# microsoft/CoCosNet

Measured on AMD Instinct MI355X. Metric: images/sec fwd+bwd ADE20k 256x256 batch-8/GPU (correspondence hot path), higher is better.
Workload: dtype f32 (K2 products as 3-term f16 hi/lo split on the f16 MFMA, fp32 accumulate); 1 GPU; ADE20k 256x256 batch 8/GPU, 64x64 grid (HW=4096), K=256, Cv=154 (rgb+151 labels), match_kernel 1, PONO_C, T=0.01; precision=f16x3; scope=hotpath: theta/phi 1x1 conv + centre/L2norm + fused corr-softmax-warp fwd+bwd; global_batch=8, parallelism=dp1, grad_payload=path, grad_allreduce_bytes=0

## Files before the change

### cocosnet_amd/csrc/split_f16.hip

```cpp
#include "common.h"

namespace cocos {

typedef _Float16 f16x4 __attribute__((ext_vector_type(4)));
typedef _Float16 f16x8 __attribute__((ext_vector_type(8)));

__device__ __forceinline__ void split1(float x, _Float16& hi, _Float16& lo) {
    hi = (_Float16)x;
    lo = (_Float16)(x - (float)hi);
}

__device__ __forceinline__ float scale_from_amax(float amax);

__global__ __launch_bounds__(256) void split_f16_flat_kernel(const float* __restrict__ x,
                                                             _Float16* __restrict__ hi,
                                                             _Float16* __restrict__ lo, size_t n4, size_t n,
                                                             float scale, const float* __restrict__ amax_dev,
                                                             float* __restrict__ scale_out) {
    const size_t i = (size_t)blockIdx.x * 256 + threadIdx.x;
    if (amax_dev) {
        scale = scale_from_amax(*amax_dev);
        if (scale_out && i == 0) *scale_out = scale;
    }
    if (i < n4) {
// ... 66 lines not shown
                if (c0 + cbase + e < Cpad) { hrow[c0 + cbase + e] = h[e]; lrow[c0 + cbase + e] = l[e]; }
        }
    }
}

__global__ __launch_bounds__(256) void split_f16_transpose_kernel(const float* __restrict__ x, _Float16* __restrict__ hi,
                                                                  _Float16* __restrict__ lo, int C, int N, int Cpad, float scale,
                                                                  const float* __restrict__ amax_dev,
                                                                  float* __restrict__ scale_out) {
    split_f16_transpose_tile(x, hi, lo, C, N, Cpad, scale, amax_dev, scale_out, blockIdx.z);
}

struct SplitPair {
    const float* x[2];
    _Float16 *hi[2], *lo[2];
    const float* amax[2];
    float* scale_out[2];
};
__global__ __launch_bounds__(256) void split_f16_transpose_pair_kernel(const SplitPair sp, int B, int C, int N, int Cpad) {
    const bool second = (int)blockIdx.z >= B;
    split_f16_transpose_tile(second ? sp.x[1] : sp.x[0], second ? sp.hi[1] : sp.hi[0], second ? sp.lo[1] : sp.lo[0], C, N, Cpad, 1.0f,
                             second ? sp.amax[1] : sp.amax[0], second ? sp.scale_out[1] : sp.scale_out[0],
                             (int)blockIdx.z - (second ? B : 0));
}

}

namespace cocos {

__global__ __launch_bounds__(256) void split_f16_rows_kernel(const float* __restrict__ x, _Float16* __restrict__ hi,
                                                             _Float16* __restrict__ lo, int rows, int cols,
                                                             int cols_pad, float scale,
                                                             const float* __restrict__ amax_dev,
                                                             float* __restrict__ scale_out) {
    const size_t i = (size_t)blockIdx.x * 256 + threadIdx.x;
    if (amax_dev) {
        scale = scale_from_amax(*amax_dev);
        if (scale_out && i == 0) *scale_out = scale;
    }
    if (i >= (size_t)rows * cols_pad) return;
    const int r = (int)(i / cols_pad), c = (int)(i - (size_t)r * cols_pad);
    _Float16 a = (_Float16)0.f, b = (_Float16)0.f;
    if (c < cols) split1(x[(size_t)r * cols + c] * scale, a, b);
    hi[i] = a;
    lo[i] = b;
}
// ... 63 lines not shown

extern "C" int cocos_split_f16_transpose_pair(const float* x0, void* hi0, void* lo0, const float* amax0_dev, float* scale0_out_dev,
                                              const float* x1, void* hi1, void* lo1, const float* amax1_dev, float* scale1_out_dev,
                                              int B, int C, int N, int Cpad, cocos_stream_t stream) {
    using namespace cocos;
    COCOS_REQUIRE(x0 && hi0 && lo0 && amax0_dev && scale0_out_dev && x1 && hi1 && lo1 && amax1_dev && scale1_out_dev, COCOS_ERR_INVALID,
                  "split_f16_transpose_pair: null pointer");
    COCOS_REQUIRE(B >= 1 && C >= 1 && N >= 1 && 2 * B <= 65535 && Cpad >= C && (Cpad + 63) / 64 <= 65535, COCOS_ERR_INVALID,
                  "split_f16_transpose_pair: bad dims B=%d C=%d N=%d Cpad=%d", B, C, N, Cpad);
    for (const void* p : {(const void*)hi0, (const void*)lo0, (const void*)hi1, (const void*)lo1})
        COCOS_REQUIRE(aligned16(p), COCOS_ERR_INVALID, "split_f16_transpose_pair: planes must be 16-byte aligned");
    SplitPair sp;
    sp.x[0] = x0; sp.x[1] = x1;
    sp.hi[0] = static_cast<_Float16*>(hi0); sp.hi[1] = static_cast<_Float16*>(hi1);
    sp.lo[0] = static_cast<_Float16*>(lo0); sp.lo[1] = static_cast<_Float16*>(lo1);
    sp.amax[0] = amax0_dev; sp.amax[1] = amax1_dev;
    sp.scale_out[0] = scale0_out_dev; sp.scale_out[1] = scale1_out_dev;
    hipLaunchKernelGGL(split_f16_transpose_pair_kernel, dim3((N + 63) / 64, (Cpad + 63) / 64, 2 * B), dim3(256), 0, as_stream(stream), sp,
                       B, C, N, Cpad);
    COCOS_HIP_CHECK(hipGetLastError());
    return COCOS_OK;
}

extern "C" int cocos_split_f16_rows(const float* x, void* hi, void* lo, int rows, int cols, int cols_pad, float scale,
                                    const float* amax_dev, float* scale_out_dev, cocos_stream_t stream) {
    using namespace cocos;
    COCOS_REQUIRE(x && hi && lo, COCOS_ERR_INVALID, "split_f16_rows: null pointer");
    COCOS_REQUIRE(rows >= 1 && cols >= 1 && cols_pad >= cols, COCOS_ERR_INVALID,
                  "split_f16_rows: bad dims rows=%d cols=%d cols_pad=%d", rows, cols, cols_pad);
    const size_t n = (size_t)rows * cols_pad;
    COCOS_REQUIRE((n + 255) / 256 <= 0x7fffffffull, COCOS_ERR_UNSUPPORTED, "split_f16_rows: tensor too large");
    hipLaunchKernelGGL(split_f16_rows_kernel, dim3((unsigned)((n + 255) / 256)), dim3(256), 0, as_stream(stream), x,
                       static_cast<_Float16*>(hi), static_cast<_Float16*>(lo), rows, cols, cols_pad, scale, amax_dev,
                       scale_out_dev);
    COCOS_HIP_CHECK(hipGetLastError());
    return COCOS_OK;
}

extern "C" int cocos_f16_plane_block_mask(const void* plane, int B, int C, int N, unsigned* mask_inout_dev,
                                          cocos_stream_t stream) {
    using namespace cocos;
    COCOS_REQUIRE(plane && mask_inout_dev, COCOS_ERR_INVALID, "f16_plane_block_mask: null pointer");
    COCOS_REQUIRE(B >= 1 && C >= 1 && C <= 1024 && N >= 1 && (long long)B * C <= 0x7fffffffll, COCOS_ERR_INVALID,
                  "f16_plane_block_mask: bad dims B=%d C=%d N=%d (C <= 1024)", B, C, N);
    hipLaunchKernelGGL(f16_plane_block_mask_kernel, dim3((unsigned)(B * C)), dim3(256), 0, as_stream(stream),
                       static_cast<const _Float16*>(plane), C, N, mask_inout_dev);
// ... 4 lines not shown
```

### cocosnet_amd/csrc/warp_values.hip

```cpp
#include <algorithm>

#include "common.h"

namespace cocos {

__global__ __launch_bounds__(256) void warp_values_kernel(const float* __restrict__ img, const float* __restrict__ seg,
                                                          float* __restrict__ out, int Ci, int Cs, int h, int w, int d,
                                                          size_t n, bool vec4, unsigned* __restrict__ amax) {
  float vmax = 0.f;
  const size_t stride = (size_t)gridDim.x * 256;
  const int W = w * d, H = h * d;
  constexpr int U = 4;
  for (size_t i0 = (size_t)blockIdx.x * 256 + threadIdx.x; i0 < n; i0 += stride * U) {
    float v[U];
    const float* pimg[U];
    bool is_img[U], live[U];
#pragma unroll
    for (int u = 0; u < U; ++u) {
      const size_t i = i0 + (size_t)u * stride;
      live[u] = i < n;
      const size_t ii = live[u] ? i : 0;
      const int x = (int)(ii % w);
      size_t r = ii / w;
      const int y = (int)(r % h);
      r /= h;
      const int c = (int)(r % (Ci + Cs));
      const size_t b = r / (Ci + Cs);
      is_img[u] = c < Ci;
      pimg[u] = nullptr;
      v[u] = 0.f;
      if (!is_img[u]) {
        v[u] = seg[((b * Cs + (c - Ci)) * H + (size_t)y * d) * W + (size_t)x * d];
      } else {
        pimg[u] = img + ((b * Ci + c) * H + (size_t)y * d) * W + (size_t)x * d;
      }
    }
#pragma unroll
    for (int u = 0; u < U; ++u) {
      if (is_img[u]) {
        const float* p = pimg[u];
        float acc = 0.f;
        if (vec4) {
#pragma unroll
          for (int a = 0; a < 4; ++a) {
            const f32x4 q = *reinterpret_cast<const f32x4*>(p + (size_t)a * W);
            acc += (q[0] + q[1]) + (q[2] + q[3]);
          }
        } else {
          for (int a = 0; a < d; ++a)
            for (int e = 0; e < d; ++e) acc += p[(size_t)a * W + e];
        }
        v[u] = acc / (float)(d * d);
      }
      if (live[u]) {
        out[i0 + (size_t)u * stride] = v[u];
        vmax = fmaxf(vmax, fabsf(v[u]));
      }
    }
  }
  if (amax) {
      __shared__ float red[4];
      vmax = wave_max_dpp(vmax);
      if ((threadIdx.x & 63) == 0) red[threadIdx.x >> 6] = vmax;
      __syncthreads();
      if (threadIdx.x == 0) atomicMax(amax, __float_as_uint(fmaxf(fmaxf(red[0], red[1]), fmaxf(red[2], red[3]))));
  }
}

__global__ __launch_bounds__(256) void warp_values_patch_kernel(const float* __restrict__ img, const float* __restrict__ seg,
                                                                float* __restrict__ out, int Ci, int Cs, int h, int w, int d,
                                                                size_t n, unsigned* __restrict__ amax) {
  float vmax = 0.f;
  const size_t stride = (size_t)gridDim.x * 256;
  const int W = w * d, H = h * d, Cp = Ci * d * d;
  for (size_t i = (size_t)blockIdx.x * 256 + threadIdx.x; i < n; i += stride) {
    const int x = (int)(i % w);
    size_t r = i / w;
    const int y = (int)(r % h);
    r /= h;
    const int c = (int)(r % (Cp + Cs));
    const size_t b = r / (Cp + Cs);
    float v;
    if (c < Cp) {
      const int cc = c / (d * d), ij = c - cc * d * d, a = ij / d, e = ij - a * d;
      v = img[((b * Ci + cc) * H + (size_t)y * d + a) * W + (size_t)x * d + e];
    } else {
      v = seg[((b * Cs + (c - Cp)) * H + (size_t)y * d) * W + (size_t)x * d];
    }
    out[i] = v;
    vmax = fmaxf(vmax, fabsf(v));
  }
  if (amax) {
      __shared__ float red[4];
      vmax = wave_max_dpp(vmax);
      if ((threadIdx.x & 63) == 0) red[threadIdx.x >> 6] = vmax;
      __syncthreads();
      if (threadIdx.x == 0) atomicMax(amax, __float_as_uint(fmaxf(fmaxf(red[0], red[1]), fmaxf(red[2], red[3]))));
  }
}

}

static int warp_values_impl(const float* img, const float* seg, float* out, int B, int Ci, int Cs, int H, int W, int down,
                            float* amax_inout_dev, cocos_stream_t stream) {
    using namespace cocos;
    COCOS_REQUIRE(out && (img || Ci == 0) && (seg || Cs == 0), COCOS_ERR_INVALID, "warp_values: null pointer");
    COCOS_REQUIRE(B >= 1 && Ci >= 0 && Cs >= 0 && Ci + Cs >= 1 && H >= 1 && W >= 1 && down >= 1, COCOS_ERR_INVALID,
                  "warp_values: bad dims B=%d Ci=%d Cs=%d H=%d W=%d down=%d", B, Ci, Cs, H, W, down);
    COCOS_REQUIRE(H % down == 0 && W % down == 0, COCOS_ERR_UNSUPPORTED,
                  "warp_values: %dx%d is not a multiple of down=%d", H, W, down);
    const size_t n = (size_t)B * (Ci + Cs) * (H / down) * (W / down);
    COCOS_REQUIRE((n + 255) / 256 <= 0x7fffffffull, COCOS_ERR_UNSUPPORTED, "warp_values: tensor too large");
    const bool vec4 = down == 4 && W % 4 == 0 && img && aligned16(img);
    const size_t blocks = std::min<size_t>(1024, (n + 1023) / 1024);
    hipLaunchKernelGGL(warp_values_kernel, dim3((unsigned)blocks), dim3(256), 0, as_stream(stream), img, seg,
                       out, Ci, Cs, H / down, W / down, down, n, vec4, reinterpret_cast<unsigned*>(amax_inout_dev));
    COCOS_HIP_CHECK(hipGetLastError());
    return COCOS_OK;
}

extern "C" int cocos_warp_values(const float* img, const float* seg, float* out, int B, int Ci, int Cs, int H, int W,
                                 int down, cocos_stream_t stream) {
    return warp_values_impl(img, seg, out, B, Ci, Cs, H, W, down, nullptr, stream);
}

extern "C" int cocos_warp_values_amax(const float* img, const float* seg, float* out, int B, int Ci, int Cs, int H, int W,
                                      int down, float* amax_inout_dev, cocos_stream_t stream) {
    COCOS_REQUIRE(amax_inout_dev, COCOS_ERR_INVALID, "warp_values_amax: null amax cell");
    return warp_values_impl(img, seg, out, B, Ci, Cs, H, W, down, amax_inout_dev, stream);
}

extern "C" int cocos_warp_values_patch_amax(const float* img, const float* seg, float* out, int B, int Ci, int Cs, int H, int W,
                                            int down, float* amax_inout_dev, cocos_stream_t stream) {
    using namespace cocos;
    COCOS_REQUIRE(out && (img || Ci == 0) && (seg || Cs == 0), COCOS_ERR_INVALID, "warp_values_patch: null pointer");
    COCOS_REQUIRE(B >= 1 && Ci >= 0 && Cs >= 0 && Ci + Cs >= 1 && H >= 1 && W >= 1 && down >= 1 && down <= 64, COCOS_ERR_INVALID,
                  "warp_values_patch: bad dims B=%d Ci=%d Cs=%d H=%d W=%d down=%d", B, Ci, Cs, H, W, down);
    COCOS_REQUIRE(H % down == 0 && W % down == 0, COCOS_ERR_UNSUPPORTED,
                  "warp_values_patch: %dx%d is not a multiple of down=%d", H, W, down);
    const size_t n = (size_t)B * ((size_t)Ci * down * down + Cs) * (H / down) * (W / down);
    COCOS_REQUIRE((size_t)Ci * down * down + Cs <= 0x7fffffffull && (n + 255) / 256 <= 0x7fffffffull, COCOS_ERR_UNSUPPORTED,
                  "warp_values_patch: tensor too large");
    const size_t blocks = std::min<size_t>(2048, (n + 255) / 256);
    hipLaunchKernelGGL(warp_values_patch_kernel, dim3((unsigned)blocks), dim3(256), 0, as_stream(stream), img, seg, out, Ci, Cs,
                       H / down, W / down, down, n, reinterpret_cast<unsigned*>(amax_inout_dev));
    COCOS_HIP_CHECK(hipGetLastError());
    return COCOS_OK;
}
```

### cocosnet_amd/ops.py

```python
from __future__ import annotations

import ctypes
import os
import sys
import threading
import weakref

import torch

from . import _lib

_C = _lib.CONSTANTS
CENTER_POSITIONS, CENTER_CHANNELS, CENTER_NONE = _C["COCOS_CENTER_POSITIONS"], _C["COCOS_CENTER_CHANNELS"], _C["COCOS_CENTER_NONE"]
NORM_EPS = sys.float_info.epsilon
MAX_FUSED_CV = 160
MAX_FUSED_SPLIT_CV = 159
MAX_DS_WORKSPACE_BYTES = 16 << 30
MAX_SAVED_LOGITS_BYTES = int(os.environ.get("COCOS_MAX_SAVED_LOGITS_BYTES", 16 << 30))
RECOMPUTE_CHUNK_BYTES = int(os.environ.get("COCOS_RECOMPUTE_CHUNK_BYTES", 1 << 30))
BWD_D_PRECOMPUTED = True
FUSED_K = 256
PRECISION = os.environ.get("COCOS_PRECISION", "f16x3")
PROJ_PRECISION = os.environ.get("COCOS_PROJ_PRECISION", "f16x3")
VALUE_LO_SKIP = True
FWD_QK_AHEAD = bool(_lib.CONSTANTS["COCOS_FWD_QK_AHEAD_DEFAULT"])
PROJ_STREAM = True
SPLIT_OPERAND_SCALE = 16.0
MATCH_FUSED = True


def _stream():
    return torch.cuda.current_stream().cuda_stream


def _select_fwd_schedule():
    _lib.load().cocos_corr_fwd_f16x3_qk_ahead(1 if FWD_QK_AHEAD else 0)


class KernelTimer:

    active = None

    def __init__(self, tags=None):
        self.events = {}
        self.tags = None if tags is None else frozenset(tags)

    def __enter__(self):
        KernelTimer.active = self
# ... 207 lines not shown
    shape = (B, N, C) if transpose else (B, C, N)
    hi = torch.empty(shape, device=x.device, dtype=torch.float16)
    lo = torch.empty(shape, device=x.device, dtype=torch.float16)
    _call("split_f16", "cocos_split_f16", x.data_ptr(), hi.data_ptr(), lo.data_ptr(), B, C, N, int(bool(transpose)),
          float(scale), _stream())
    return hi, lo


def split_f16_chan_mask(x: torch.Tensor, amax: torch.Tensor, want_mask: bool):
    x = _chk(x, "split_f16_chan_mask: x")
    B, C, N = x.shape
    if N % 4 != 0 or C > 1024 or x.data_ptr() % 16 != 0:
        hi, lo, sc = split_f16(x, False, amax=amax)
        return hi, lo, sc, (f16_plane_block_mask(lo) if want_mask else None)
    hi = torch.empty((B, C, N), device=x.device, dtype=torch.float16)
    lo = torch.empty((B, C, N), device=x.device, dtype=torch.float16)
    sc = torch.empty(1, device=x.device, dtype=torch.float32)
    mask = _zero_cell(x.device) if want_mask else None
    _call("split_f16", "cocos_split_f16_chan_mask", x.data_ptr(), hi.data_ptr(), lo.data_ptr(), B, C, N, amax.data_ptr(),
          sc.data_ptr(), _ptr(mask), _stream())
    return hi, lo, sc, mask


def f16_plane_block_mask(plane: torch.Tensor) -> torch.Tensor:
    B, C, N = plane.shape
    cell = _zero_cell(plane.device)
    _call("f16_plane_block_mask", "cocos_f16_plane_block_mask", plane.data_ptr(), B, C, N, cell.data_ptr(), _stream())
    return cell


def _recompute_chunk(B, Nq, Nk):
    per_key = max(B * Nq * 4, 1)
    nchunks = max(1, -(-(per_key * Nk) // max(RECOMPUTE_CHUNK_BYTES, 1)))
    kc = max(128, -(-Nk // nchunks) // 128 * 128 + (128 if (-(-Nk // nchunks)) % 128 else 0))
    return min(kc, (Nk + 127) // 128 * 128)


def _saves_logits(B, Nq, Nk) -> bool:
    return (B * Nq * Nk * 4 <= MAX_SAVED_LOGITS_BYTES
            and _lib.load().cocos_corr_softmax_warp_saved_logits_bytes(1, Nq, Nk) < 2 ** 31 - 1)


def _split_bwd_ok(B, Nq, Nk, Cv):
    if not (Nk % 8 == 0 and Nq % 8 == 0 and Cv <= MAX_FUSED_CV):
        return False
    if _saves_logits(B, Nq, Nk):
# ... 11 lines not shown
    while bmode == 2 and tiles * S < GEMM_SPLIT_K_BELOW and S < 8 and Kred % (64 * S) == 0:
        S *= 2
    if S == 1:
        _call(timer, "cocos_hgemm_f16x3", ah.data_ptr(), al.data_ptr(), bh.data_ptr(), bl.data_ptr(), out.data_ptr(), B, M, n, Kred,
              host, _ptr(dev1), _ptr(dev2), bmode, st)
        return
    a2h = ah.view(B, M, S, Kred // S).transpose(1, 2).contiguous()
    a2l = al.view(B, M, S, Kred // S).transpose(1, 2).contiguous()
    part = torch.empty((B, S, M, n), device=out.device, dtype=torch.float32)
    _call(timer, "cocos_hgemm_f16x3", a2h.data_ptr(), a2l.data_ptr(), bh.data_ptr(), bl.data_ptr(), part.data_ptr(), B * S, M, n,
          Kred // S, host, _ptr(dev1), _ptr(dev2), bmode, st)
    torch.sum(part, dim=1, out=out)


def _key_gemm(qch, qcl, dsh, dsl, dk, n, Nq, k_active, qks, ds_scale, gemm_b, st):
    K = dk.shape[1]
    assert qch.shape[1] == K and (not k_active or k_active == K)
    _hgemm_planes("corr_softmax_warp_bwd_key_from_ds", qch, qcl, dsh, dsl, dk, K, n, Nq, 1.0 if qks else 1.0 / SPLIT_OPERAND_SCALE,
                  ds_scale, qks[0] if qks else None, gemm_b, st)


class _CorrSoftmaxWarp(torch.autograd.Function):
    @staticmethod
    def forward(ctx, qn, kn, v, inv_temperature: float, keep_logits: bool, planes=None):
        qn, kn, v = _chk(qn, "qn"), _chk(kn, "kn"), _chk(v, "v")
        B, K, Nq = qn.shape
        Bk, Kk, Nk = kn.shape
        Bv, Cv, Nv = v.shape
        if (Bk, Kk) != (B, K) or (Bv, Nv) != (B, Nk):
            raise ValueError(f"corr_softmax_warp: shape mismatch qn{tuple(qn.shape)} "
                             f"kn{tuple(kn.shape)} v{tuple(v.shape)}")
        out = torch.empty((B, Cv, Nq), device=qn.device, dtype=torch.float32)
        lse = torch.empty((B, Nq), device=qn.device, dtype=torch.float32)
        logits_t = None
        ctx.split = planes is not None
        ctx.v_amax = None
        ctx.v_lomask = None
        if planes is not None:
            qh, ql, kh, kl, vh, vl, v_scale, v_amax, v_lomask = planes[:9]
            qk_scales = planes[13] if len(planes) > 13 else None
            ctx.k_active = planes[14] if len(planes) > 14 else 0
            Kp = FUSED_K if ctx.k_active else K
            ctx.recompute = bool(keep_logits) and not _saves_logits(B, Nq, Nk)
            if keep_logits and not ctx.recompute:
                nbytes = _lib.load().cocos_corr_softmax_warp_saved_logits_bytes(B, Nq, Nk)
                logits_t = torch.empty(nbytes // 4, device=qn.device, dtype=torch.float32)
            ctx.rowstat = torch.empty((B, 3, Nq), device=qn.device, dtype=torch.float32) if (qk_scales and keep_logits) else None
            ctx.mtile = (torch.empty((B, (Nk + 31) // 32, 2, Nq), device=qn.device, dtype=torch.float32)
                         if (qk_scales and logits_t is not None) else None)
            _select_fwd_schedule()
            _call("corr_softmax_warp_fwd", "cocos_corr_softmax_warp_fwd_f16x3_ex", qh.data_ptr(), ql.data_ptr(),
                  kh.data_ptr(), kl.data_ptr(), vh.data_ptr(), vl.data_ptr(), out.data_ptr(), lse.data_ptr(),
                  _ptr(logits_t), v_scale.data_ptr(), _ptr(v_lomask), B, Kp, Nq, Nk, Cv, float(inv_temperature),
                  SPLIT_OPERAND_SCALE, _ptr(qk_scales[0] if qk_scales else None), _ptr(qk_scales[1] if qk_scales else None),
                  _ptr(ctx.rowstat), _ptr(ctx.mtile), ctx.k_active, _stream())
            ctx.v_amax = v_amax
            ctx.v_lomask = v_lomask
            ctx.qk_scales = qk_scales
        else:
            keep = (keep_logits and B * Nq * Nk * 4 <= MAX_DS_WORKSPACE_BYTES and Nq * Nk * 4 < 2 ** 31 - 1)
            logits_t = torch.empty((B, Nk, Nq), device=qn.device, dtype=torch.float32) if keep else None
            _call("corr_softmax_warp_fwd", "cocos_corr_softmax_warp_fwd", qn.data_ptr(), kn.data_ptr(),
                  v.data_ptr(), out.data_ptr(), lse.data_ptr(), _ptr(logits_t), B, K, Nq, Nk, Cv,
                  float(inv_temperature), _stream())
        ctx.save_for_backward(qn, kn, v, out, lse)
        ctx.logits_t = logits_t
        ctx.inv_t = float(inv_temperature)
        recompute = planes is not None and getattr(ctx, "recompute", False)
        ctx.cplanes = planes[9:13] if (planes is not None and len(planes) > 9 and (logits_t is not None or recompute)) else None
        ctx.pplanes = planes[0:4] if recompute else None
        return out

    @staticmethod
    def backward(ctx, dout):
        qn, kn, v, out, lse = ctx.saved_tensors
        dout = _chk(dout, "dout")
        B, K, Nq = qn.shape
        Nk, Cv = kn.shape[2], v.shape[1]
        need_q, need_k, need_v = ctx.needs_input_grad[:3]
        dqn = torch.empty_like(qn) if need_q else None
        dkn = torch.empty_like(kn) if (need_k or need_v) else None
        dv = torch.empty_like(v) if need_v else None
        st = _stream()
        logits_t = ctx.logits_t
        if ctx.split and getattr(ctx, "recompute", False):
            return _CorrSoftmaxWarp._backward_recompute(ctx, qn, kn, v, out, lse, dout, dqn, dkn, dv, need_k)
        if ctx.split and logits_t is not None:
            qch, qcl, kch, kcl = ctx.cplanes
            qks = ctx.qk_scales
            cvp = (Cv + 31) // 32 * 32
            g_amax, v_amax = _recall_amax(dout), ctx.v_amax
            if g_amax is None:
                g_amax = absmax(dout)
            (gph, gpl, g_scale), (vph, vpl, v_scale) = _split_pair_transposed(dout, g_amax, v, v_amax, cvp)
            half = dict(device=qn.device, dtype=torch.float16)
            want_k = dkn is not None
            dsh = dsl = psh = psl = None
            if want_k:
                dsh, dsl = torch.empty((B, Nk, Nq), **half), torch.empty((B, Nk, Nq), **half)
            if dv is not None:
                psh, psl = torch.empty((B, Nk, Nq), **half), torch.empty((B, Nk, Nq), **half)
            ds_scale = torch.empty(1, device=qn.device, dtype=torch.float32)
            blocked = int(Nk % 128 == 0 and Nq % 32 == 0)
            gemm_b = 2 * blocked
            ka = getattr(ctx, "k_active", 0)
            Kp = FUSED_K if ka else K
            if ka:
                dqn_buf = torch.empty((B, Kp, Nq), device=qn.device, dtype=torch.float32)
                dqn = dqn_buf[:, :K] if dqn is not None else None
            elif dqn is None:
                dqn_buf = torch.empty_like(qn)
            else:
                dqn_buf = dqn
            d_pre = _rowdot_cached(dout, out) if BWD_D_PRECOMPUTED else None
            _call("corr_softmax_warp_bwd_query", "cocos_corr_softmax_warp_bwd_query_f16x3_ex", kch.data_ptr(),
                  kcl.data_ptr(), vph.data_ptr(), vpl.data_ptr(), gph.data_ptr(), gpl.data_ptr(),
                  g_scale.data_ptr(), out.data_ptr(), dout.data_ptr(), lse.data_ptr(), logits_t.data_ptr(),
                  dqn_buf.data_ptr(), _ptr(dsh), _ptr(dsl), _ptr(psh), _ptr(psl), v_amax.data_ptr(),
                  v_scale.data_ptr(), ds_scale.data_ptr(), _ptr(ctx.v_lomask), B, Kp, Nq, Nk, Cv, cvp, ctx.inv_t,
                  SPLIT_OPERAND_SCALE, _ptr(qks[0] if qks else None), _ptr(qks[1] if qks else None), blocked,
                  _ptr(getattr(ctx, "rowstat", None)), _ptr(getattr(ctx, "mtile", None)), _ptr(d_pre), ka, st)
            if want_k:
                _key_gemm(qch, qcl, dsh, dsl, dkn, Nk, Nq, ka, qks, ds_scale, gemm_b, st)
            if dv is not None:
                gch, gcl, _ = split_f16(dout, False, amax=g_amax)
                _hgemm_planes("corr_softmax_warp_bwd_dv", gch, gcl, psh, psl, dv, Cv, Nk, Nq, 1.0 / 16384.0, g_scale, None, gemm_b, st)
            return dqn, (dkn if need_k else None), dv, None, None, None
        ds_bytes = B * Nq * Nk * 4
        via_gemm = (dqn is not None and dkn is not None and dv is None
                    and ds_bytes <= MAX_DS_WORKSPACE_BYTES and Nq * Nk * 4 < 2 ** 31 - 1)
        key_recompute = dkn is not None and not via_gemm
        dvec = None
        if key_recompute or (dqn is not None and logits_t is None):
            dvec = torch.empty((B, Nq), device=qn.device, dtype=torch.float32)
            _call("corr_softmax_warp_bwd_prepare", "cocos_corr_softmax_warp_bwd_prepare",
                  out.data_ptr(), dout.data_ptr(), dvec.data_ptr(), B, Nq, Cv, st)
        dims = (B, K, Nq, Nk, Cv, ctx.inv_t, st)
        ds_t = torch.empty((B, Nk, Nq), device=qn.device, dtype=torch.float32) if via_gemm else None
        if dqn is not None:
            _call("corr_softmax_warp_bwd_query", "cocos_corr_softmax_warp_bwd_query", qn.data_ptr(),
                  kn.data_ptr(), v.data_ptr(), out.data_ptr(), lse.data_ptr(), dout.data_ptr(),
                  _ptr(dvec), _ptr(logits_t), _ptr(dqn), _ptr(ds_t), *dims)
        if via_gemm:
            _call("corr_softmax_warp_bwd_key_from_ds", "cocos_corr_softmax_warp_bwd_key_from_ds",
                  qn.data_ptr(), ds_t.data_ptr(), dkn.data_ptr(), B, K, Nq, Nk, st)
        elif dkn is not None:
            _call("corr_softmax_warp_bwd_key", "cocos_corr_softmax_warp_bwd_key", qn.data_ptr(),
                  kn.data_ptr(), v.data_ptr(), lse.data_ptr(), dout.data_ptr(), dvec.data_ptr(),
                  _ptr(dkn), _ptr(dv), *dims)
        return dqn, (dkn if need_k else None), dv, None, None, None


def _corr_bwd_recompute(ctx, qn, kn, v, out, lse, dout, dqn, dkn, dv, need_k):
    qh, ql, kh, kl = ctx.pplanes
    qch, qcl, kch, kcl = ctx.cplanes
    qks = ctx.qk_scales
    B, K, Nq = qn.shape
    Nk, Cv = kn.shape[2], v.shape[1]
    st = _stream()
    lib = _lib.load()
    cvp = (Cv + 31) // 32 * 32
    g_amax, v_amax = _recall_amax(dout), ctx.v_amax
    if g_amax is None:
        g_amax = absmax(dout)
    gph, gpl, g_scale = split_f16(dout, True, cpad=cvp, amax=g_amax)
    vph, vpl, v_scale = split_f16(v, True, cpad=cvp, amax=v_amax)
    gch = gcl = None
    if dv is not None:
        gch, gcl, _ = split_f16(dout, False, amax=g_amax)
    dev, half = qn.device, dict(device=qn.device, dtype=torch.float16)
    want_k = dkn is not None
    kc = _recompute_chunk(B, Nq, Nk)
    ds_scale = torch.empty(1, device=dev, dtype=torch.float32)
# ... 24 lines not shown
        blocked = int(n % 128 == 0 and Nq % 32 == 0)
        dq_c = torch.empty((B, Kp, Nq), device=dev, dtype=torch.float32)
        _call("corr_softmax_warp_bwd_query", "cocos_corr_softmax_warp_bwd_query_f16x3_ex", kchc.data_ptr(), kclc.data_ptr(),
              vphc.data_ptr(), vplc.data_ptr(), gph.data_ptr(), gpl.data_ptr(), g_scale.data_ptr(), out.data_ptr(), dout.data_ptr(),
              lse.data_ptr(), lg.data_ptr(), dq_c.data_ptr(), _ptr(dsh), _ptr(dsl), _ptr(psh), _ptr(psl), v_amax.data_ptr(),
              v_scale.data_ptr(), ds_scale.data_ptr(), _ptr(ctx.v_lomask), B, Kp, Nq, n, Cv, cvp, ctx.inv_t, SPLIT_OPERAND_SCALE,
              _ptr(qks[0] if qks else None), _ptr(qks[1] if qks else None), blocked, _ptr(rowstat), _ptr(mt), _ptr(d_pre), ka, st)
        del lg
        if ka:
            dq_c = dq_c[:, :K]
        dq_acc = dq_c if dq_acc is None else dq_acc.add_(dq_c)
        if want_k:
            dk_c = dkn if n == Nk else torch.empty((B, K, n), device=dev, dtype=torch.float32)
            _key_gemm(qch, qcl, dsh, dsl, dk_c, n, Nq, ka, qks, ds_scale, 2 * blocked, st)
            if dk_c is not dkn:
                dkn[:, :, k0:k0 + n] = dk_c
        if dv is not None:
            dv_c = dv if n == Nk else torch.empty((B, Cv, n), device=dev, dtype=torch.float32)
            _hgemm_planes("corr_softmax_warp_bwd_dv", gch, gcl, psh, psl, dv_c, Cv, n, Nq, 1.0 / 16384.0, g_scale, None, 2 * blocked, st)
            if dv_c is not dv:
                dv[:, :, k0:k0 + n] = dv_c
    if dqn is not None:
        dqn = dq_acc
    return dqn, (dkn if need_k else None), dv, None, None, None


_CorrSoftmaxWarp._backward_recompute = staticmethod(_corr_bwd_recompute)


def _rowdot(a: torch.Tensor, b: torch.Tensor) -> torch.Tensor:
    B, C, N = a.shape
    d = torch.empty((B, N), device=a.device, dtype=torch.float32)
    _call("rowdot", "cocos_rowdot_f64", a.data_ptr(), b.data_ptr(), d.data_ptr(), B, C, N, _stream())
    return d


def _rowdot_cached(dout: torch.Tensor, out: torch.Tensor):
    ent, _tls.known_rowdot = _tls.known_rowdot, None
    if ent is not None:
        ref, version, out_ptr, d = ent
        src = ref()
        if (src is not None and src.data_ptr() == dout.data_ptr() and src.shape == dout.shape and dout._version == version
                and out.data_ptr() == out_ptr and dout.is_contiguous()):
            return d
    return _rowdot(dout, out)


# ... 37 lines not shown
    if not split and (planes.has(qn) or planes.has(kn)):
        raise _lib.CocosHipError("corr_softmax_warp: qn / kn exist as operand planes only (center_l2norm_planes) but this "
                                 "shape does not take the split-precision kernels")

    qk_made = []

    def qk_planes():
        if not qk_made:
            qa, ka_ = absmax(qn), absmax(kn)
            qh, ql, qs = split_f16(qn, True, cpad=FUSED_K, amax=qa)
            kh, kl, ks = split_f16(kn, True, cpad=FUSED_K, amax=ka_)
            cpl = (None,) * 4
            if keep:
                qch, qcl, _ = split_f16(qn, False, amax=qa)
                kch, kcl, _ = split_f16(kn, False, amax=ka_)
                if K < FUSED_K:
                    pad = lambda t: torch.cat([t, t.new_zeros((B, FUSED_K - K, Nk))], dim=1)
                    kch, kcl = pad(kch), pad(kcl)
                cpl = (qch, qcl, kch, kcl)
            qk_made.append((qh, ql, kh, kl, *cpl, (qs, ks), K if K < FUSED_K else 0))
        return qk_made[0]

    def run(vv):
        pl = None
        if split:
            with torch.no_grad():
                v_amax = _recall_amax(vv)
                if v_amax is None:
                    v_amax = absmax(vv)
                vh, vl, v_scale, v_lomask = split_f16_chan_mask(vv, v_amax, VALUE_LO_SKIP and vv.shape[1] > 32 and not operand_amax)
                if operand_amax:
                    pl = (*qk_planes()[:4], vh, vl, v_scale, v_amax, v_lomask, *qk_planes()[4:])
                else:
                    pl = (*planes.get(qn, True, SPLIT_OPERAND_SCALE), *planes.get(kn, True, SPLIT_OPERAND_SCALE),
                          vh, vl, v_scale, v_amax, v_lomask)
                    if keep:
                        pl += (*planes.get(qn, False, SPLIT_OPERAND_SCALE), *planes.get(kn, False, SPLIT_OPERAND_SCALE))
        return _CorrSoftmaxWarp.apply(qn, kn, vv, inv_temperature, keep, pl)

    limit = MAX_FUSED_SPLIT_CV if split else MAX_FUSED_CV
    if Cv <= limit:
        return run(v)
    return torch.cat([run(v[:, c0:c0 + limit]) for c0 in range(0, Cv, limit)], dim=1)


class PreparedValues:

    def __init__(self, v: torch.Tensor, n_ref: int):
        self.v, self.n_ref = v, int(n_ref)
        self.amax = None
        self._split = None
        self._expanded = {}

    def split(self):
        if self._split is None:
            self.amax = absmax(self.v)
            self._split = split_f16_chan_mask(self.v, self.amax, VALUE_LO_SKIP and self.v.shape[1] > 32)
        return self._split

    def expanded(self, B: int) -> torch.Tensor:
        Be = self.v.shape[0]
# ... 3218 lines not shown
```

### include/cocos_hip.h

```cpp
#ifndef COCOS_HIP_H
#define COCOS_HIP_H

#include <stddef.h>
#include <stdint.h>

#ifdef __cplusplus
extern "C" {
#endif

#define COCOS_OK 0
#define COCOS_ERR_INVALID (-1)
#define COCOS_ERR_UNSUPPORTED (-2)
#define COCOS_ERR_HIP (-3)
#define COCOS_ERR_WORKSPACE (-4)

typedef void* cocos_stream_t;

int cocos_version(void);
const char* cocos_last_error_string(void);

#define COCOS_CENTER_POSITIONS 0
#define COCOS_CENTER_CHANNELS 1
#define COCOS_CENTER_NONE 2
int cocos_center_l2norm_fwd(const float* x, float* y, float* norm, float* row_ws,
// ... 242 lines not shown
int cocos_warp_head_bwd(const float* g_img, const float* g_mask, const float* o, float* dout, float* drow, float* amax_inout_dev,
                        int B, int Ci, int Cs, int h, int w, int down, cocos_stream_t stream);
#define COCOS_WARP_HEAD_NEAREST 0
#define COCOS_WARP_HEAD_BILINEAR 1
#define COCOS_WARP_HEAD_PATCH 2
int cocos_warp_head_fwd_ex(const float* o, float* y, float* y_bi, int B, int Ci, int C, int h, int w, int down, int mode,
                           cocos_stream_t stream);
int cocos_warp_head_bwd_ex(const float* g_img, const float* g_mask, const float* g_y, const float* o, float* dout, float* drow,
                           float* amax_inout_dev, int B, int Ci, int Cs, int h, int w, int down, int mode, cocos_stream_t stream);
float cocos_warp_head_bilinear_tap(int down, int idx, int first, int last);

int cocos_warp_values(const float* img, const float* seg, float* out, int B, int Ci, int Cs, int H, int W,
                      int down, cocos_stream_t stream);
int cocos_warp_values_amax(const float* img, const float* seg, float* out, int B, int Ci, int Cs, int H, int W,
                           int down, float* amax_inout_dev, cocos_stream_t stream);
int cocos_warp_values_patch_amax(const float* img, const float* seg, float* out, int B, int Ci, int Cs, int H, int W,
                                 int down, float* amax_inout_dev, cocos_stream_t stream);

int cocos_concat2_amax(const float* a, const float* b, float* out, int B, long long na, long long nb,
                       float* amax_inout_dev , cocos_stream_t stream);
int cocos_split_f16_chan_mask(const float* x, void* hi, void* lo, int B, int C, int N, const float* amax_dev,
                              float* scale_out_dev , unsigned* mask_inout_dev ,
                              cocos_stream_t stream);
int cocos_proj_weight_planes(const float* w, void* rows_hi, void* rows_lo, void* t_hi ,
                             void* t_lo , int Cout, int Cin, int KpadIn, int KpadOut, const float* amax_dev,
                             float* scale_out_dev , cocos_stream_t stream);

int cocos_sum_leading(const float* x, float* out, int S, long long n, cocos_stream_t stream);
int cocos_channel_sum_slices(int C, long long N);
int cocos_channel_sum(const float* dy, float* db, float* partials, int B, int C, long long N, cocos_stream_t stream);
int cocos_box3_stat_grads(const float* r1, const float* r2, const float* c1, const float* c2, const float* a, const float* b,
                          float* dmu, float* dnu, float* da, float* db, long long n, float k_unfolded, float scale,
                          cocos_stream_t stream);

int cocos_logits_softmax_warp_fwd_f16x3(const float* logits_t, const void* vh, const void* vl, float* out, float* lse,
                                        const float* v_scale_dev , int B, int Nq, int Nk, int Cv,
                                        cocos_stream_t stream);
int cocos_logits_softmax_warp_bwd_f16x3(const float* logits_t, const void* vph, const void* vpl, const void* gph,
                                        const void* gpl, const float* g_scale_dev, const float* v_scale_dev ,
                                        const float* out, const float* dout, const float* lse, float* dlogits_t, int B,
                                        int Nq, int Nk, int Cv, int CvPad, cocos_stream_t stream);

int cocos_contextual_rows_fwd(const float* cosm, float* cx, long long rows, int cols, float h, float eps,
                              cocos_stream_t stream);
int cocos_contextual_rows_bwd(const float* cosm, const float* dcx, float* dcos, long long rows, int cols, float h,
                              float eps, cocos_stream_t stream);
// ... 311 lines not shown
```

Before: 7132 images/s.

## Emit transposed value planes in forward split and row-vectorise label gather

The forward value split now also writes the position-major (transposed) hi/lo planes in the same kernel through a shared-memory tile. These planes are saved for backward, so backward only has to split dout instead of re-reading v to build the transposed pair. Separately, warp_values with down=4 now handles the label channels a whole row per wave with vectorised loads, and the amax atomic is skipped when it would not raise the stored value. The cost is extra memory held between forward and backward and more complex dispatch conditions.

```diff
diff --git a/cocosnet_amd/csrc/split_f16.hip b/cocosnet_amd/csrc/split_f16.hip
--- a/cocosnet_amd/csrc/split_f16.hip
+++ b/cocosnet_amd/csrc/split_f16.hip
@@ -112,6 +112,65 @@
     split_f16_transpose_tile(second ? sp.x[1] : sp.x[0], second ? sp.hi[1] : sp.hi[0], second ? sp.lo[1] : sp.lo[0], C, N, Cpad, 1.0f,
                              second ? sp.amax[1] : sp.amax[0], second ? sp.scale_out[1] : sp.scale_out[0],
                              (int)blockIdx.z - (second ? B : 0));
+}
+
+__global__ __launch_bounds__(256) void split_f16_chan_mask_both_kernel(const float* __restrict__ x, _Float16* __restrict__ hi,
+                                                                       _Float16* __restrict__ lo, _Float16* __restrict__ thi,
+                                                                       _Float16* __restrict__ tlo, int C, int N, int Cpad,
+                                                                       const float* __restrict__ amax_dev,
+                                                                       float* __restrict__ scale_out,
+                                                                       unsigned* __restrict__ mask) {
+    __shared__ float tile[64][65];
+    const int tid = threadIdx.x, b = blockIdx.z;
+    const int c0 = blockIdx.y * 64, n0 = blockIdx.x * 64;
+    const size_t plane = (size_t)b * C * N;
+    const float scale = scale_from_amax(*amax_dev);
+    if (tid == 0 && blockIdx.x == 0 && blockIdx.y == 0 && b == 0) *scale_out = scale;
+    {
+        const int q = tid & 15, r = tid >> 4;
+        unsigned bits = 0;
+#pragma unroll
+        for (int u = 0; u < 4; ++u) {
+            const int ch = c0 + r + 16 * u, n = n0 + 4 * q;
+            f32x4 v = {0.f, 0.f, 0.f, 0.f};
+            if (ch < C && n < N) {
+                const size_t at = plane + (size_t)ch * N + n;
+                v = *reinterpret_cast<const f32x4*>(x + at) * scale;
+                f16x4 h, l;
+#pragma unroll
+                for (int e = 0; e < 4; ++e) { _Float16 a, c; split1(v[e], a, c); h[e] = a; l[e] = c; }
+                *reinterpret_cast<f16x4*>(hi + at) = h;
+                *reinterpret_cast<f16x4*>(lo + at) = l;
+                typedef unsigned int u32x2_t __attribute__((ext_vector_type(2)));
+                const u32x2_t w = __builtin_bit_cast(u32x2_t, l);
+                if (((w.x | w.y) & 0x7fff7fffu) != 0u) bits |= 1u << (ch >> 5);
+            }
+#pragma unroll
+            for (int e = 0; e < 4; ++e) tile[r + 16 * u][4 * q + e] = v[e];
+        }
+        if (mask && bits != 0u && (__builtin_nontemporal_load(mask) & bits) != bits) atomicOr(mask, bits);
+    }
+    __syncthreads();
+    const int p = tid >> 2, cq = tid & 3;
+    const int n = n0 + p;
+    if (n >= N) return;
+    _Float16* hrow = thi + ((size_t)b * N + n) * Cpad;
+    _Float16* lrow = tlo + ((size_t)b * N + n) * Cpad;
+#pragma unroll
+    for (int g = 0; g < 2; ++g) {
+        const int cbase = cq * 16 + g * 8;
+        f16x8 h, l;
+#pragma unroll
+        for (int e = 0; e < 8; ++e) { _Float16 a, c; split1(tile[cbase + e][p], a, c); h[e] = a; l[e] = c; }
+        if (c0 + cbase + 8 <= Cpad && (Cpad % 8) == 0) {
+            *reinterpret_cast<f16x8*>(hrow + c0 + cbase) = h;
+            *reinterpret_cast<f16x8*>(lrow + c0 + cbase) = l;
+        } else {
+#pragma unroll
+            for (int e = 0; e < 8; ++e)
+                if (c0 + cbase + e < Cpad) { hrow[c0 + cbase + e] = h[e]; lrow[c0 + cbase + e] = l[e]; }
+        }
+    }
 }
 
 }
@@ -221,6 +280,26 @@
     return COCOS_OK;
 }
 
+extern "C" int cocos_split_f16_chan_mask_both(const float* x, void* hi, void* lo, void* t_hi, void* t_lo, int B, int C, int N,
+                                              int Cpad, const float* amax_dev, float* scale_out_dev, unsigned* mask_inout_dev,
+                                              cocos_stream_t stream) {
+    using namespace cocos;
+    COCOS_REQUIRE(x && hi && lo && t_hi && t_lo && amax_dev && scale_out_dev, COCOS_ERR_INVALID,
+                  "split_f16_chan_mask_both: null pointer");
+    COCOS_REQUIRE(B >= 1 && C >= 1 && N >= 1 && Cpad >= C, COCOS_ERR_INVALID,
+                  "split_f16_chan_mask_both: bad dims B=%d C=%d N=%d Cpad=%d", B, C, N, Cpad);
+    COCOS_REQUIRE(N % 4 == 0 && C <= 1024 && B <= 65535 && (Cpad + 63) / 64 <= 65535, COCOS_ERR_UNSUPPORTED,
+                  "split_f16_chan_mask_both: needs N %% 4 == 0, C <= 1024, B <= 65535 (B=%d C=%d N=%d Cpad=%d)", B, C, N, Cpad);
+    COCOS_REQUIRE(aligned16(x) && (reinterpret_cast<uintptr_t>(hi) & 7u) == 0 && (reinterpret_cast<uintptr_t>(lo) & 7u) == 0 &&
+                      aligned16(t_hi) && aligned16(t_lo),
+                  COCOS_ERR_INVALID, "split_f16_chan_mask_both: x and the position-major planes must be 16-byte, the channel-major planes 8-byte aligned");
+    hipLaunchKernelGGL(split_f16_chan_mask_both_kernel, dim3((N + 63) / 64, (Cpad + 63) / 64, B), dim3(256), 0, as_stream(stream),
+                       x, static_cast<_Float16*>(hi), static_cast<_Float16*>(lo), static_cast<_Float16*>(t_hi),
+                       static_cast<_Float16*>(t_lo), C, N, Cpad, amax_dev, scale_out_dev, mask_inout_dev);
+    COCOS_HIP_CHECK(hipGetLastError());
+    return COCOS_OK;
+}
+
 extern "C" int cocos_split_f16_rows(const float* x, void* hi, void* lo, int rows, int cols, int cols_pad, float scale,
                                     const float* amax_dev, float* scale_out_dev, cocos_stream_t stream) {
     using namespace cocos;
diff --git a/cocosnet_amd/csrc/warp_values.hip b/cocosnet_amd/csrc/warp_values.hip
--- a/cocosnet_amd/csrc/warp_values.hip
+++ b/cocosnet_amd/csrc/warp_values.hip
@@ -3,6 +3,90 @@
 #include "common.h"
 
 namespace cocos {
+
+__device__ __forceinline__ float wv_window_mean(const float* __restrict__ p, int W, int d, bool vec4) {
+  float acc = 0.f;
+  if (vec4) {
+#pragma unroll
+    for (int a = 0; a < 4; ++a) {
+      const f32x4 q = *reinterpret_cast<const f32x4*>(p + (size_t)a * W);
+      acc += (q[0] + q[1]) + (q[2] + q[3]);
+    }
+  } else {
+    for (int a = 0; a < d; ++a)
+      for (int e = 0; e < d; ++e) acc += p[(size_t)a * W + e];
+  }
+  return acc / (float)(d * d);
+}
+
+__device__ __forceinline__ void wv_block_amax(float vmax, unsigned* __restrict__ amax) {
+  __shared__ float red[4];
+  vmax = wave_max_dpp(vmax);
+  if ((threadIdx.x & 63) == 0) red[threadIdx.x >> 6] = vmax;
+  __syncthreads();
+  if (threadIdx.x == 0) {
+    const unsigned m = __float_as_uint(fmaxf(fmaxf(red[0], red[1]), fmaxf(red[2], red[3])));
+    if (__builtin_nontemporal_load(amax) < m) atomicMax(amax, m);
+  }
+}
+
+template <int U>
+__device__ __forceinline__ float wv_label_rows4(const float* __restrict__ seg, float* __restrict__ out, int Cs, int Ctot,
+                                                int coff, int h, int w, unsigned rows) {
+  const int lane = threadIdx.x & 63;
+  const unsigned wave = blockIdx.x * 4u + (threadIdx.x >> 6), nwaves = gridDim.x * 4u;
+  const size_t W = (size_t)w * 4;
+  float vmax = 0.f;
+  for (unsigned r0 = wave * U; r0 < rows; r0 += nwaves * U) {
+    const unsigned pc0 = r0 / (unsigned)h, y0 = r0 - pc0 * (unsigned)h;
+    const unsigned b0 = pc0 / (unsigned)Cs, c0 = pc0 - b0 * (unsigned)Cs;
+    for (int x0 = 0; x0 < w; x0 += 64) {
+      const int x = x0 + lane;
+      f32x4 q[U];
+#pragma unroll
+      for (int u = 0; u < U; ++u) {
+        q[u] = f32x4{0.f, 0.f, 0.f, 0.f};
+        if (r0 + u < rows && x < w) q[u] = *reinterpret_cast<const f32x4*>(seg + (size_t)(r0 + u) * 4 * W + (size_t)x * 4);
+      }
+      unsigned y = y0, c = c0, b = b0;
+#pragma unroll
+      for (int u = 0; u < U; ++u) {
+        asm volatile("" : "+v"(q[u]));
+        if (r0 + u < rows && x < w) {
+          out[(((size_t)b * Ctot + coff + c) * h + y) * w + x] = q[u][0];
+          vmax = fmaxf(vmax, fabsf(q[u][0]));
+        }
+        if (++y == (unsigned)h) {
+          y = 0;
+          if (++c == (unsigned)Cs) { c = 0; ++b; }
+        }
+      }
+    }
+  }
+  return vmax;
+}
+
+__global__ __launch_bounds__(256) void warp_values_rows_kernel(const float* __restrict__ img, const float* __restrict__ seg,
+                                                               float* __restrict__ out, int Ci, int Cs, int h, int w, int B,
+                                                               bool vec4, unsigned* __restrict__ amax) {
+  constexpr int d = 4;
+  const int W = w * d, H = h * d;
+  float vmax = 0.f;
+  const size_t n_img = (size_t)B * Ci * h * w, stride = (size_t)gridDim.x * 256;
+  for (size_t i = (size_t)blockIdx.x * 256 + threadIdx.x; i < n_img; i += stride) {
+    const int x = (int)(i % w);
+    size_t r = i / w;
+    const int y = (int)(r % h);
+    r /= h;
+    const int c = (int)(r % Ci);
+    const size_t b = r / Ci;
+    const float v = wv_window_mean(img + ((b * Ci + c) * H + (size_t)y * d) * W + (size_t)x * d, W, d, vec4);
+    out[((b * (Ci + Cs) + c) * h + y) * w + x] = v;
+    vmax = fmaxf(vmax, fabsf(v));
+  }
+  vmax = fmaxf(vmax, wv_label_rows4<4>(seg, out, Cs, Ci + Cs, Ci, h, w, (unsigned)B * Cs * h));
+  if (amax) wv_block_amax(vmax, amax);
+}
 
 __global__ __launch_bounds__(256) void warp_values_kernel(const float* __restrict__ img, const float* __restrict__ seg,
                                                           float* __restrict__ out, int Ci, int Cs, int h, int w, int d,
@@ -37,49 +121,31 @@
     }
 #pragma unroll
     for (int u = 0; u < U; ++u) {
-      if (is_img[u]) {
-        const float* p = pimg[u];
-        float acc = 0.f;
-        if (vec4) {
-#pragma unroll
-          for (int a = 0; a < 4; ++a) {
-            const f32x4 q = *reinterpret_cast<const f32x4*>(p + (size_t)a * W);
-            acc += (q[0] + q[1]) + (q[2] + q[3]);
-          }
-        } else {
-          for (int a = 0; a < d; ++a)
-            for (int e = 0; e < d; ++e) acc += p[(size_t)a * W + e];
-        }
-        v[u] = acc / (float)(d * d);
-      }
+      if (is_img[u]) v[u] = wv_window_mean(pimg[u], W, d, vec4);
       if (live[u]) {
         out[i0 + (size_t)u * stride] = v[u];
         vmax = fmaxf(vmax, fabsf(v[u]));
       }
     }
   }
-  if (amax) {
-      __shared__ float red[4];
-      vmax = wave_max_dpp(vmax);
-      if ((threadIdx.x & 63) == 0) red[threadIdx.x >> 6] = vmax;
-      __syncthreads();
-      if (threadIdx.x == 0) atomicMax(amax, __float_as_uint(fmaxf(fmaxf(red[0], red[1]), fmaxf(red[2], red[3]))));
-  }
+  if (amax) wv_block_amax(vmax, amax);
 }
 
 __global__ __launch_bounds__(256) void warp_values_patch_kernel(const float* __restrict__ img, const float* __restrict__ seg,
                                                                 float* __restrict__ out, int Ci, int Cs, int h, int w, int d,
-                                                                size_t n, unsigned* __restrict__ amax) {
+                                                                int B, bool rows4, unsigned* __restrict__ amax) {
   float vmax = 0.f;
   const size_t stride = (size_t)gridDim.x * 256;
   const int W = w * d, H = h * d, Cp = Ci * d * d;
+  const int Ce = rows4 ? Cp : Cp + Cs;
+  const size_t n = (size_t)B * Ce * h * w;
   for (size_t i = (size_t)blockIdx.x * 256 + threadIdx.x; i < n; i += stride) {
     const int x = (int)(i % w);
     size_t r = i / w;
     const int y = (int)(r % h);
     r /= h;
-    const int c = (int)(r % (Cp + Cs));
-    const size_t b = r / (Cp + Cs);
+    const int c = (int)(r % Ce);
+    const size_t b = r / Ce;
     float v;
     if (c < Cp) {
       const int cc = c / (d * d), ij = c - cc * d * d, a = ij / d, e = ij - a * d;
@@ -87,16 +153,19 @@
     } else {
       v = seg[((b * Cs + (c - Cp)) * H + (size_t)y * d) * W + (size_t)x * d];
     }
-    out[i] = v;
+    out[((b * (Cp + Cs) + c) * h + y) * w + x] = v;
     vmax = fmaxf(vmax, fabsf(v));
   }
-  if (amax) {
-      __shared__ float red[4];
-      vmax = wave_max_dpp(vmax);
-      if ((threadIdx.x & 63) == 0) red[threadIdx.x >> 6] = vmax;
-      __syncthreads();
-      if (threadIdx.x == 0) atomicMax(amax, __float_as_uint(fmaxf(fmaxf(red[0], red[1]), fmaxf(red[2], red[3]))));
-  }
+  if (rows4) vmax = fmaxf(vmax, wv_label_rows4<4>(seg, out, Cs, Cp + Cs, Cp, h, w, (unsigned)B * Cs * h));
+  if (amax) wv_block_amax(vmax, amax);
+}
+
+#ifndef COCOS_WV_ROWS_MAX_BLOCKS
+#define COCOS_WV_ROWS_MAX_BLOCKS 4096
+#endif
+static size_t wv_rows_blocks(size_t rows, size_t n_elem) {
+  const size_t want = std::max((rows + 15) / 16, (n_elem + 1023) / 1024);
+  return std::max<size_t>(1, std::min<size_t>(COCOS_WV_ROWS_MAX_BLOCKS, want));
 }
 
 }
@@ -112,9 +181,15 @@
     const size_t n = (size_t)B * (Ci + Cs) * (H / down) * (W / down);
     COCOS_REQUIRE((n + 255) / 256 <= 0x7fffffffull, COCOS_ERR_UNSUPPORTED, "warp_values: tensor too large");
     const bool vec4 = down == 4 && W % 4 == 0 && img && aligned16(img);
-    const size_t blocks = std::min<size_t>(1024, (n + 1023) / 1024);
-    hipLaunchKernelGGL(warp_values_kernel, dim3((unsigned)blocks), dim3(256), 0, as_stream(stream), img, seg,
-                       out, Ci, Cs, H / down, W / down, down, n, vec4, reinterpret_cast<unsigned*>(amax_inout_dev));
+    if (down == 4 && Cs > 0 && aligned16(seg) && (size_t)B * Cs * (H / 4) < 0x7fffffffull) {
+        const size_t blocks = wv_rows_blocks((size_t)B * Cs * (H / 4), (size_t)B * Ci * (H / 4) * (W / 4));
+        hipLaunchKernelGGL(warp_values_rows_kernel, dim3((unsigned)blocks), dim3(256), 0, as_stream(stream), img, seg, out, Ci,
+                           Cs, H / 4, W / 4, B, vec4, reinterpret_cast<unsigned*>(amax_inout_dev));
+    } else {
+        const size_t blocks = std::min<size_t>(1024, (n + 1023) / 1024);
+        hipLaunchKernelGGL(warp_values_kernel, dim3((unsigned)blocks), dim3(256), 0, as_stream(stream), img, seg,
+                           out, Ci, Cs, H / down, W / down, down, n, vec4, reinterpret_cast<unsigned*>(amax_inout_dev));
+    }
     COCOS_HIP_CHECK(hipGetLastError());
     return COCOS_OK;
 }
@@ -141,9 +216,12 @@
     const size_t n = (size_t)B * ((size_t)Ci * down * down + Cs) * (H / down) * (W / down);
     COCOS_REQUIRE((size_t)Ci * down * down + Cs <= 0x7fffffffull && (n + 255) / 256 <= 0x7fffffffull, COCOS_ERR_UNSUPPORTED,
                   "warp_values_patch: tensor too large");
-    const size_t blocks = std::min<size_t>(2048, (n + 255) / 256);
+    const bool rows4 = down == 4 && Cs > 0 && aligned16(seg) && (size_t)B * Cs * (H / 4) < 0x7fffffffull;
+    const size_t hw = (size_t)(H / down) * (W / down);
+    const size_t blocks = rows4 ? wv_rows_blocks((size_t)B * Cs * (H / 4), (size_t)B * Ci * 16 * hw)
+                                : std::min<size_t>(2048, (n + 255) / 256);
     hipLaunchKernelGGL(warp_values_patch_kernel, dim3((unsigned)blocks), dim3(256), 0, as_stream(stream), img, seg, out, Ci, Cs,
-                       H / down, W / down, down, n, reinterpret_cast<unsigned*>(amax_inout_dev));
+                       H / down, W / down, down, B, rows4, reinterpret_cast<unsigned*>(amax_inout_dev));
     COCOS_HIP_CHECK(hipGetLastError());
     return COCOS_OK;
 }
diff --git a/cocosnet_amd/ops.py b/cocosnet_amd/ops.py
--- a/cocosnet_amd/ops.py
+++ b/cocosnet_amd/ops.py
@@ -24,6 +24,7 @@
 PROJ_PRECISION = os.environ.get("COCOS_PROJ_PRECISION", "f16x3")
 VALUE_LO_SKIP = True
 FWD_QK_AHEAD = bool(_lib.CONSTANTS["COCOS_FWD_QK_AHEAD_DEFAULT"])
+VALUE_PLANES_FWD = os.environ.get("COCOS_VALUE_PLANES_FWD", "1") != "0"
 PROJ_STREAM = True
 SPLIT_OPERAND_SCALE = 16.0
 MATCH_FUSED = True
@@ -277,6 +278,21 @@
     return hi, lo, sc, mask
 
 
+def split_f16_chan_mask_both(x: torch.Tensor, amax: torch.Tensor, want_mask: bool, cpad: int):
+    x = _chk(x, "split_f16_chan_mask_both: x")
+    B, C, N = x.shape
+    if N % 4 != 0 or C > 1024 or B > 65535 or x.data_ptr() % 16 != 0:
+        return (*split_f16_chan_mask(x, amax, want_mask), None, None)
+    half = dict(device=x.device, dtype=torch.float16)
+    hi, lo = torch.empty((B, C, N), **half), torch.empty((B, C, N), **half)
+    thi, tlo = torch.empty((B, N, int(cpad)), **half), torch.empty((B, N, int(cpad)), **half)
+    sc = torch.empty(1, device=x.device, dtype=torch.float32)
+    mask = _zero_cell(x.device) if want_mask else None
+    _call("split_f16", "cocos_split_f16_chan_mask_both", x.data_ptr(), hi.data_ptr(), lo.data_ptr(), thi.data_ptr(), tlo.data_ptr(),
+          B, C, N, int(cpad), amax.data_ptr(), sc.data_ptr(), _ptr(mask), _stream())
+    return hi, lo, sc, mask, thi, tlo
+
+
 def f16_plane_block_mask(plane: torch.Tensor) -> torch.Tensor:
     B, C, N = plane.shape
     cell = _zero_cell(plane.device)
@@ -334,7 +350,7 @@
 
 class _CorrSoftmaxWarp(torch.autograd.Function):
     @staticmethod
-    def forward(ctx, qn, kn, v, inv_temperature: float, keep_logits: bool, planes=None):
+    def forward(ctx, qn, kn, v, inv_temperature: float, keep_logits: bool, planes=None, v_tplanes=None):
         qn, kn, v = _chk(qn, "qn"), _chk(kn, "kn"), _chk(v, "v")
         B, K, Nq = qn.shape
         Bk, Kk, Nk = kn.shape
@@ -381,6 +397,7 @@
         recompute = planes is not None and getattr(ctx, "recompute", False)
         ctx.cplanes = planes[9:13] if (planes is not None and len(planes) > 9 and (logits_t is not None or recompute)) else None
         ctx.pplanes = planes[0:4] if recompute else None
+        ctx.v_tplanes = v_tplanes if (planes is not None and logits_t is not None) else None
         return out
 
     @staticmethod
@@ -404,7 +421,11 @@
             g_amax, v_amax = _recall_amax(dout), ctx.v_amax
             if g_amax is None:
                 g_amax = absmax(dout)
-            (gph, gpl, g_scale), (vph, vpl, v_scale) = _split_pair_transposed(dout, g_amax, v, v_amax, cvp)
+            if ctx.v_tplanes is not None:
+                vph, vpl, v_scale = ctx.v_tplanes
+                gph, gpl, g_scale = split_f16(dout, True, cpad=cvp, amax=g_amax)
+            else:
+                (gph, gpl, g_scale), (vph, vpl, v_scale) = _split_pair_transposed(dout, g_amax, v, v_amax, cvp)
             half = dict(device=qn.device, dtype=torch.float16)
             want_k = dkn is not None
             dsh = dsl = psh = psl = None
@@ -437,7 +458,7 @@
             if dv is not None:
                 gch, gcl, _ = split_f16(dout, False, amax=g_amax)
                 _hgemm_planes("corr_softmax_warp_bwd_dv", gch, gcl, psh, psl, dv, Cv, Nk, Nq, 1.0 / 16384.0, g_scale, None, gemm_b, st)
-            return dqn, (dkn if need_k else None), dv, None, None, None
+            return dqn, (dkn if need_k else None), dv, None, None, None, None
         ds_bytes = B * Nq * Nk * 4
         via_gemm = (dqn is not None and dkn is not None and dv is None
                     and ds_bytes <= MAX_DS_WORKSPACE_BYTES and Nq * Nk * 4 < 2 ** 31 - 1)
@@ -460,7 +481,7 @@
             _call("corr_softmax_warp_bwd_key", "cocos_corr_softmax_warp_bwd_key", qn.data_ptr(),
                   kn.data_ptr(), v.data_ptr(), lse.data_ptr(), dout.data_ptr(), dvec.data_ptr(),
                   _ptr(dkn), _ptr(dv), *dims)
-        return dqn, (dkn if need_k else None), dv, None, None, None
+        return dqn, (dkn if need_k else None), dv, None, None, None, None
 
 
 def _corr_bwd_recompute(ctx, qn, kn, v, out, lse, dout, dqn, dkn, dv, need_k):
@@ -531,7 +552,7 @@
                 dv[:, :, k0:k0 + n] = dv_c
     if dqn is not None:
         dqn = dq_acc
-    return dqn, (dkn if need_k else None), dv, None, None, None
+    return dqn, (dkn if need_k else None), dv, None, None, None, None
 
 
 _CorrSoftmaxWarp._backward_recompute = staticmethod(_corr_bwd_recompute)
@@ -615,13 +636,19 @@
         return qk_made[0]
 
     def run(vv):
-        pl = None
+        pl = v_t = None
         if split:
             with torch.no_grad():
                 v_amax = _recall_amax(vv)
                 if v_amax is None:
                     v_amax = absmax(vv)
-                vh, vl, v_scale, v_lomask = split_f16_chan_mask(vv, v_amax, VALUE_LO_SKIP and vv.shape[1] > 32 and not operand_amax)
+                want_mask = VALUE_LO_SKIP and vv.shape[1] > 32 and not operand_amax
+                if VALUE_PLANES_FWD and keep and not operand_amax and vv is v and _saves_logits(B, Nq, Nk):
+                    vh, vl, v_scale, v_lomask, vph, vpl = split_f16_chan_mask_both(vv, v_amax, want_mask, (Cv + 31) // 32 * 32)
+                    if vph is not None:
+                        v_t = (vph, vpl, v_scale)
+                else:
+                    vh, vl, v_scale, v_lomask = split_f16_chan_mask(vv, v_amax, want_mask)
                 if operand_amax:
                     pl = (*qk_planes()[:4], vh, vl, v_scale, v_amax, v_lomask, *qk_planes()[4:])
                 else:
@@ -629,7 +656,7 @@
                           vh, vl, v_scale, v_amax, v_lomask)
                     if keep:
                         pl += (*planes.get(qn, False, SPLIT_OPERAND_SCALE), *planes.get(kn, False, SPLIT_OPERAND_SCALE))
-        return _CorrSoftmaxWarp.apply(qn, kn, vv, inv_temperature, keep, pl)
+        return _CorrSoftmaxWarp.apply(qn, kn, vv, inv_temperature, keep, pl, v_t)
 
     limit = MAX_FUSED_SPLIT_CV if split else MAX_FUSED_CV
     if Cv <= limit:
diff --git a/include/cocos_hip.h b/include/cocos_hip.h
--- a/include/cocos_hip.h
+++ b/include/cocos_hip.h
@@ -288,6 +288,9 @@
 int cocos_split_f16_chan_mask(const float* x, void* hi, void* lo, int B, int C, int N, const float* amax_dev,
                               float* scale_out_dev , unsigned* mask_inout_dev ,
                               cocos_stream_t stream);
+int cocos_split_f16_chan_mask_both(const float* x, void* hi, void* lo, void* t_hi, void* t_lo, int B, int C, int N, int Cpad,
+                                   const float* amax_dev, float* scale_out_dev, unsigned* mask_inout_dev ,
+                                   cocos_stream_t stream);
 int cocos_proj_weight_planes(const float* w, void* rows_hi, void* rows_lo, void* t_hi ,
                              void* t_lo , int Cout, int Cin, int KpadIn, int KpadOut, const float* amax_dev,
                              float* scale_out_dev , cocos_stream_t stream);
```

Result: no change. 7186 images/s (median of 6 runs) (+0.8%).
